# Roy-Shubhajit/FIT-GNN

Measured on AMD Instinct MI355X. Metric: edges aggregated/sec (GCN fwd+bwd) on coarsened subgraphs, higher is better.
Workload: dtype f32

## Files before the change

### fit-gnn_amd/csrc/gcn_ops.hip

```cpp
#include <hip/hip_runtime.h>
#include <stdint.h>

#include <algorithm>

#include "common.h"
#include "fitgnn_hip.h"

namespace {

__global__ void gcn_deg_kernel(const int32_t *__restrict__ rowptr, const float *__restrict__ w, float *__restrict__ dinv,
                               int32_t n_rows) {
    const int i = blockIdx.x * blockDim.x + threadIdx.x;
    if (i >= n_rows) return;
    const int e0 = rowptr[i], e1 = rowptr[i + 1];
    float d = 0.f;
    if (w) {
        for (int e = e0; e < e1; ++e) d += w[e];
    } else {
        d = (float)(e1 - e0);
    }
    dinv[i] = d > 0.f ? 1.0f / sqrtf(d) : 0.f;
}

__global__ void gcn_val_kernel(const int32_t *__restrict__ rowptr, const int32_t *__restrict__ col,
// ... 73 lines not shown
                for (int u = 0; u < U; ++u) nz[u] = __ballot((__float_as_uint(dyl[u]) & 0x7fffffffu) != 0u) != 0ull;
            }
#pragma unroll
            for (int u = 0; u < U; ++u) {
                const int row = min(row0 + 4 * u, r1 - 1);
                const int64_t base = ((sel && !compact_in) ? sel[row] : (int64_t)row) * H + col0;
                if (HEAD && !nz[u]) {
#pragma unroll
                    for (int i = 0; i < VEC; ++i) o[u][i] = 0.f;
                    continue;
                }
                if (VEC == 4) {
                    const float4 ov = *reinterpret_cast<const float4 *>(out + base);
                    o[u][0] = ov.x; o[u][1 % VEC] = ov.y; o[u][2 % VEC] = ov.z; o[u][3 % VEC] = ov.w;
                    if (!HEAD) {
                        const float4 gv = *reinterpret_cast<const float4 *>(dOut + base);
                        g[u][0] = gv.x; g[u][1 % VEC] = gv.y; g[u][2 % VEC] = gv.z; g[u][3 % VEC] = gv.w;
                    }
                } else {
                    o[u][0] = out[base];
                    if (!HEAD) g[u][0] = dOut[base];
                }
            }
#pragma unroll
            for (int u = 0; u < U; ++u) {
                const int row = row0 + 4 * u;
                if (row >= r1) break;
                const int64_t zbase = (int64_t)row * H + col0;
                const int64_t base = (sel ? sel[row] : (int64_t)row) * H + col0;
                if (HEAD && !nz[u]) {
                    if (VEC == 4) {
                        *reinterpret_cast<float4 *>(dZ + zbase) = make_float4(0.f, 0.f, 0.f, 0.f);
                    } else {
                        dZ[zbase] = 0.f;
                    }
                    continue;
                }
                if (HEAD) {
#pragma unroll
                    for (int i = 0; i < VEC; ++i) g[u][i] = 0.f;
                    for (int c = 0; c < C; ++c) {
                        const float d = __int_as_float(__builtin_amdgcn_readlane(__float_as_int(dyl[u]), c));
#pragma unroll
                        for (int i = 0; i < VEC; ++i) g[u][i] = fmaf(d, s_w[c * SLAB + lane * VEC + i], g[u][i]);
                    }
                    if (CW > 0) {
#pragma unroll
                        for (int c = 0; c < (CW > 0 ? CW : 1); ++c) {
                            const float d = __int_as_float(__builtin_amdgcn_readlane(__float_as_int(dyl[u]), c));
#pragma unroll
                            for (int i = 0; i < VEC; ++i) wacc[c][i] = fmaf(d, o[u][i], wacc[c][i]);
                        }
                    }
                }
                uint64_t bits = 0;
                if ((epi & FITGNN_EPI_DROPOUT) && !mask) bits = fitgnn::dropout_bits(seed, (uint64_t)base >> 2);
#pragma unroll
                for (int i = 0; i < VEC; ++i) {
                    float d = g[u][i];
                    if (epi & FITGNN_EPI_DROPOUT) {
                        const uint64_t idx = (uint64_t)base + i;
                        const bool keep = mask ? (mask[idx] != 0) : fitgnn::dropout_keep(bits, (int)(idx & 3), thresh);
                        d = keep ? d * scale : 0.f;
                    }
                    if (epi & FITGNN_EPI_ELU) {
                        const float e = o[u][i] * unscale;
                        d = e > 0.f ? d : d * (e + 1.0f);
// ... 849 lines not shown
```

### fit-gnn_amd/csrc/gemm_f32.hip

```cpp
#include <algorithm>
#include <cmath>

#include "common.h"
#include "fitgnn_hip.h"

namespace {

typedef float f32x16 __attribute__((ext_vector_type(16)));

constexpr int kBK = 32;
constexpr int kPitch = 36;

template <int WM, int WN, int MI, int NJ, bool AKM, bool BKM>
struct Geo {
    static constexpr int TI = 32 * MI * WM, TJ = 32 * NJ * WN, THREADS = 64 * WM * WN;
    static constexpr int A_DW = AKM ? kBK * TI : TI * kPitch;
    static constexpr int B_DW = BKM ? kBK * TJ : TJ * kPitch;
    static constexpr int STAGE_DW = A_DW + B_DW;
    static constexpr int LDS_BYTES = 2 * STAGE_DW * 4;
    static constexpr int NA = TI * 8 / THREADS, NB = TJ * 8 / THREADS;
    static_assert(LDS_BYTES <= 160 * 1024, "tile does not fit the CU's LDS");
    static_assert(TI * 8 % THREADS == 0 && TJ * 8 % THREADS == 0, "stage not divisible over the threads");
};

template <bool KM, int T, int NV, int THREADS>
__device__ __forceinline__ void load_slab(float4 (&r)[NV], const float *__restrict__ P, long ld, long t0, long lim, long k0, long klim) {
    const int tid = threadIdx.x;
#pragma unroll
    for (int p = 0; p < NV; ++p) {
        const int v = tid + p * THREADS;
        if (!KM) {
            const int row = v >> 3, k4 = v & 7;
            long i = t0 + row;
            i = i < lim ? i : lim - 1;
            const long k = k0 + 4 * k4;
            r[p] = k < klim ? *reinterpret_cast<const float4 *>(P + i * ld + k) : make_float4(0.f, 0.f, 0.f, 0.f);
        } else {
            constexpr int Q = T / 4;
            const int kr = v / Q, c4 = v % Q;
            long i = t0 + 4 * c4;
            i = i + 4 <= lim ? i : lim - 4;
            const long k = k0 + kr;
            r[p] = k < klim ? *reinterpret_cast<const float4 *>(P + k * ld + i) : make_float4(0.f, 0.f, 0.f, 0.f);
        }
// ... 9 lines not shown
        if (!KM) {
            const int row = v >> 3, k4 = v & 7;
            *reinterpret_cast<float4 *>(lds + row * kPitch + 4 * k4) = r[p];
        } else {
            constexpr int Q = T / 4;
            const int kr = v / Q, c4 = v % Q;
            *reinterpret_cast<float4 *>(lds + kr * T + 4 * c4) = r[p];
        }
    }
}

template <bool KM, int T>
__device__ __forceinline__ void frag(float (&f)[4], const float *lds, int o, int kk, int lane) {
    if (!KM) {
        const float4 v = *reinterpret_cast<const float4 *>(lds + (o + (lane & 31)) * kPitch + 8 * kk + 4 * (lane >> 5));
        f[0] = v.x; f[1] = v.y; f[2] = v.z; f[3] = v.w;
    } else {
        const float *p = lds + (8 * kk + 4 * (lane >> 5)) * T + o + (lane & 31);
#pragma unroll
        for (int s = 0; s < 4; ++s) f[s] = p[s * T];
    }
}

template <int WM, int WN, int MI, int NJ, bool AKM, bool BKM>
__global__ __launch_bounds__(64 * WM * WN) void gemm_f32_kernel(const float *__restrict__ A, long lda, const float *__restrict__ B, long ldb,
                                                                   long I, int J, long K, float *__restrict__ C, long ldc, int tiles_i,
                                                                   int tiles_j, int nchunks, long chunk_k) {
    using G = Geo<WM, WN, MI, NJ, AKM, BKM>;
    extern __shared__ __attribute__((aligned(16))) float lds_f[];
    const int lane = threadIdx.x & 63, wave = __builtin_amdgcn_readfirstlane(threadIdx.x >> 6);
    const int wm = wave / WN, wn = wave % WN;
    const int xcd = blockIdx.x & 7, slot = blockIdx.x >> 3;
    int ti, tj, chunk = 0;
    if (nchunks > 1) {
        const int ntile = tiles_i * tiles_j;
        const int tile = slot % ntile;
        chunk = xcd + 8 * (slot / ntile);
        ti = tile / tiles_j, tj = tile % tiles_j;
        if (chunk >= nchunks) return;
    } else {
        tj = slot % tiles_j;
        ti = xcd + 8 * (slot / tiles_j);
        if (ti >= tiles_i) return;
    }
    const long i0 = (long)ti * G::TI, j0 = (long)tj * G::TJ;
    const long k_begin = (long)chunk * chunk_k;
    const long k_end = nchunks > 1 ? (k_begin + chunk_k < K ? k_begin + chunk_k : K) : K;
    const int nstage = k_end > k_begin ? (int)((k_end - k_begin + kBK - 1) / kBK) : 0;

    f32x16 acc[MI][NJ];
// ... 34 lines not shown
#pragma unroll
        for (int kk = 0; kk < NKK; ++kk) {
            float fa[MI][4], fb[NJ][4];
            read_frags(fa, fb, sa, sb, kk);
            multiply(fa, fb);
        }
    };
    for (int s = 0; s < nstage; ++s) {
        const bool more = s + 1 < nstage;
        if (more) {
            const long k0 = k_begin + (long)(s + 1) * kBK;
            load_slab<AKM, G::TI, G::NA, G::THREADS>(ra, A, lda, i0, I, k0, k_end);
            load_slab<BKM, G::TJ, G::NB, G::THREADS>(rb, B, ldb, j0, (long)J, k0, k_end);
        }
        products(s);
        if (more) {
            float *na = lds_f + ((s + 1) & 1) * G::STAGE_DW;
            store_slab<AKM, G::TI, G::NA, G::THREADS>(ra, na);
            store_slab<BKM, G::TJ, G::NB, G::THREADS>(rb, na + G::A_DW);
        }
        __syncthreads();
    }

    float *out = nchunks > 1 ? C + (long)chunk * I * J : C;
    const long ldo = nchunks > 1 ? (long)J : ldc;
#pragma unroll
    for (int i = 0; i < MI; ++i) {
#pragma unroll
        for (int j = 0; j < NJ; ++j) {
            const long col = j0 + wn * (32 * NJ) + j * 32 + (lane & 31);
            const long row0 = i0 + wm * (32 * MI) + i * 32 + 4 * (lane >> 5);
#pragma unroll
            for (int r = 0; r < 16; ++r) {
                const long row = row0 + (r & 3) + 8 * (r >> 2);
                if (row < I && col < J) out[row * ldo + col] = acc[i][j][r];
            }
        }
    }
}

__global__ __launch_bounds__(256) void sum_chunks_kernel(const float *__restrict__ partial, int nchunks, long IJ, float *__restrict__ out, int J,
                                                         long ldc) {
    const long q = (long)blockIdx.x * blockDim.x + threadIdx.x;
    if (q >= IJ) return;
    float part[8];
#pragma unroll
    for (int u = 0; u < 8; ++u) part[u] = 0.f;
    int c = 0;
    for (; c + 8 <= nchunks; c += 8) {
#pragma unroll
        for (int u = 0; u < 8; ++u) part[u] += partial[(long)(c + u) * IJ + q];
    }
#pragma unroll
    for (int u = 0; u < 8; ++u)
        if (c + u < nchunks) part[u] += partial[(long)(c + u) * IJ + q];
    float acc = part[0];
#pragma unroll
    for (int u = 1; u < 8; ++u) acc += part[u];
    out[(q / J) * ldc + (q % J)] = acc;
}

enum Shape { S256 = 0, S256x128, S64x512, S128, S64x128, S128x64, S64x64 };
struct ShapeDim { int ti, tj, per_cu; };
constexpr ShapeDim kShape[] = {{256, 256, 1}, {256, 128, 1}, {64, 512, 1}, {128, 128, 2}, {64, 128, 2}, {128, 64, 2}, {64, 64, 4}};

struct Plan {
    int shape;
    int tiles_i, tiles_j, nchunks;
    long chunk_k;
    long main_rows;
    int rem_tiles_i, rem_chunks;
    long rem_chunk_k;
};

Plan make_plan(long I, int J, long K, bool akm, bool bkm) {
    Plan p;
    const bool tn = akm && bkm;
    auto tiles_of = [&](int sh) { return ((I + kShape[sh].ti - 1) / kShape[sh].ti) * ((J + kShape[sh].tj - 1) / kShape[sh].tj); };
    if (tn) {
        if (I <= 64) p.shape = S64x512;
        else if (J <= 128 || K < 65536) p.shape = S128;
        else p.shape = S256;
// ... 26 lines not shown
    for (long c = 8; c <= most && c <= 256; c += 8) {
        const double t = ceil(ntile * (double)c / slots) * t_tile / (double)c + (double)(c + 1) * (double)I * (double)J * 4.0 / 3.0e12 + 4e-6;
        if (t < 0.92 * best) { best = t; p.nchunks = (int)c; }
    }
    if (p.nchunks > 1) {
        const long per = (K + p.nchunks - 1) / p.nchunks;
        p.chunk_k = (per + kBK - 1) / kBK * kBK;
    }
    p.main_rows = 0; p.rem_tiles_i = 0; p.rem_chunks = 1; p.rem_chunk_k = K;
    const long T = (long)p.tiles_i * p.tiles_j;
    const long full = T / 256, rem = T % 256;
    if (!akm && kShape[p.shape].per_cu == 1 && p.nchunks == 1 && full >= 1 && rem > 0 && rem <= 96 && K >= 8 * 2 * kBK) {
        const long main_tiles_i = full * 256 / p.tiles_j;
        if (main_tiles_i >= 1 && main_tiles_i < p.tiles_i) {
            p.main_rows = main_tiles_i * TI;
            p.rem_tiles_i = (int)(p.tiles_i - main_tiles_i);
            p.rem_chunks = 8;
            p.rem_chunk_k = ((K + 7) / 8 + kBK - 1) / kBK * kBK;
        }
    }
    return p;
}

template <int WM, int WN, int MI, int NJ, bool AKM, bool BKM>
int launch(const Plan &p, const float *a, long lda, const float *b, long ldb, long I, int J, long K, float *c, long ldc, hipStream_t s) {
    using G = Geo<WM, WN, MI, NJ, AKM, BKM>;
    static std::atomic<uint64_t> lds_done{0};
    if (const int rc = fitgnn_lds_limit_once((const void *)gemm_f32_kernel<WM, WN, MI, NJ, AKM, BKM>, G::LDS_BYTES, lds_done)) return rc;
    unsigned grid;
    if (p.nchunks > 1) grid = (unsigned)(p.tiles_i * p.tiles_j * ((p.nchunks + 7) / 8 * 8));
    else grid = (unsigned)((p.tiles_i + 7) / 8 * 8 * p.tiles_j);
    hipLaunchKernelGGL((gemm_f32_kernel<WM, WN, MI, NJ, AKM, BKM>), dim3(grid), dim3(G::THREADS), G::LDS_BYTES, s, a, lda, b, ldb, I, J, K,
                       c, ldc, p.tiles_i, p.tiles_j, p.nchunks, p.chunk_k);
    return (int)hipGetLastError();
}

template <bool AKM, bool BKM>
int launch_shape(const Plan &p, const float *a, long lda, const float *b, long ldb, long I, int J, long K, float *c, long ldc, hipStream_t s) {
    if constexpr (AKM && BKM) {
        if (p.shape == S64x512) return launch<1, 4, 2, 4, AKM, BKM>(p, a, lda, b, ldb, I, J, K, c, ldc, s);
    }
    switch (p.shape) {
        case S256x128: return launch<4, 1, 2, 4, AKM, BKM>(p, a, lda, b, ldb, I, J, K, c, ldc, s);
        case S128: return launch<2, 2, 2, 2, AKM, BKM>(p, a, lda, b, ldb, I, J, K, c, ldc, s);
        case S64x128: return launch<2, 2, 1, 2, AKM, BKM>(p, a, lda, b, ldb, I, J, K, c, ldc, s);
        case S128x64: return launch<4, 1, 1, 2, AKM, BKM>(p, a, lda, b, ldb, I, J, K, c, ldc, s);
        case S64x64: return launch<2, 2, 1, 1, AKM, BKM>(p, a, lda, b, ldb, I, J, K, c, ldc, s);
        default: return launch<4, 2, 2, 4, AKM, BKM>(p, a, lda, b, ldb, I, J, K, c, ldc, s);
    }
}

}

extern "C" size_t fitgnn_gemm_exact_workspace_bytes(int64_t I, int32_t J, int64_t K, int32_t a_kmajor, int32_t b_kmajor) {
    if (I <= 0 || J <= 0 || K <= 0) return 0;
    const Plan p = make_plan((long)I, J, (long)K, a_kmajor != 0, b_kmajor != 0);
    if (p.main_rows > 0) return (size_t)p.rem_chunks * (size_t)(I - p.main_rows) * (size_t)J * sizeof(float);
    return p.nchunks > 1 ? (size_t)p.nchunks * (size_t)I * (size_t)J * sizeof(float) : 0;
}

extern "C" int fitgnn_gemm_exact_plan(int64_t I, int32_t J, int64_t K, int32_t a_kmajor, int32_t b_kmajor, int32_t *shape, int32_t *nchunks,
                                      int64_t *main_rows) {
    if (I <= 0 || J <= 0 || K <= 0 || !shape || !nchunks || !main_rows) return FITGNN_E_BADARG;
    const Plan p = make_plan((long)I, J, (long)K, a_kmajor != 0, b_kmajor != 0);
    *shape = p.shape;
    *nchunks = p.nchunks;
    *main_rows = p.main_rows;
    return 0;
}

extern "C" int fitgnn_gemm_exact_f32(const float *a, int64_t lda, int32_t a_kmajor, const float *b, int64_t ldb, int32_t b_kmajor,
                                     int64_t I, int32_t J, int64_t K, float *c, int64_t ldc, void *workspace, void *stream) {
// ... 27 lines not shown
        hipLaunchKernelGGL(sum_chunks_kernel, dim3((unsigned)((IJ + 255) / 256)), dim3(256), 0, s, (const float *)workspace, pr.nchunks, IJ,
                           c + p.main_rows * (long)ldc, J, (long)ldc);
        return (int)hipGetLastError();
    }
    float *dst = c;
    long ldd = (long)ldc;
    if (p.nchunks > 1) {
        if (!workspace || ((uintptr_t)workspace % 16) != 0) return FITGNN_E_BADARG;
        dst = (float *)workspace;
    }
    int rc;
    if (a_kmajor) rc = launch_shape<true, true>(p, a, (long)lda, b, (long)ldb, (long)I, J, (long)K, dst, ldd, s);
    else if (b_kmajor) rc = launch_shape<false, true>(p, a, (long)lda, b, (long)ldb, (long)I, J, (long)K, dst, ldd, s);
    else rc = launch_shape<false, false>(p, a, (long)lda, b, (long)ldb, (long)I, J, (long)K, dst, ldd, s);
    if (rc) return rc;
    if (p.nchunks > 1) {
        const long IJ = (long)I * J;
        hipLaunchKernelGGL(sum_chunks_kernel, dim3((unsigned)((IJ + 255) / 256)), dim3(256), 0, s, (const float *)workspace, p.nchunks, IJ, c, J,
                           (long)ldc);
        return (int)hipGetLastError();
    }
    return 0;
}
```

### fit-gnn_amd/fitgnn_amd/_lib.py

```python
import ctypes
import os

_HERE = os.path.dirname(os.path.abspath(__file__))
LIB_PATH = os.path.join(os.path.dirname(_HERE), "lib", "libfitgnn_hip.so")

c_i32, c_i64, c_u32, c_u64, c_f32, c_size = (ctypes.c_int32, ctypes.c_int64, ctypes.c_uint32, ctypes.c_uint64,
                                              ctypes.c_float, ctypes.c_size_t)
ptr = ctypes.c_void_p

EPI_BIAS, EPI_ELU, EPI_DROPOUT, EPI_SEED_DEVICE = 1, 2, 4, 8
SPMM_GATHER = 0x100
MAX_K = 16
MATCH_HEAVY_EDGE, MATCH_ALGEBRAIC_JC = 0, 1
MATCH_SMALL_MAX_NODES, MATCH_SMALL_MAX_NNZ, MATCH_SMALL_MAX_K, MATCH_SMALL_LDS_BUDGET = 128, 1024, 12, 65536
MATCH_DONE, MATCH_TOO_BIG, MATCH_BAD_INPUT = 1, 2, 3
QUALITY_MAX_K = 64

SIGNATURES = {
    "fitgnn_abi_version": (ctypes.c_int, []),
    "fitgnn_error_string": (ctypes.c_char_p, [ctypes.c_int]),
    "fitgnn_stream_copy_f32": (ctypes.c_int, [ptr, ptr, c_i64, ptr]),
    "fitgnn_spmm_default_window_rows": (ctypes.c_int, []),
    "fitgnn_spmm_max_window_rows": (ctypes.c_int, [c_i32]),
    "fitgnn_gcn_norm_csr_f32": (ctypes.c_int, [ptr, ptr, ptr, ptr, ptr, c_i32, ptr]),
# ... 40 lines not shown
    "fitgnn_epilogue_bwd_head_rows_f32": (ctypes.c_int, [ptr, ptr, c_i32, ptr, ptr, c_i32, c_i32, ptr, c_i32, c_u32, c_f32, c_u64, ptr,
                                                        ptr, ptr, ptr, c_size, ptr]),
    "fitgnn_epilogue_bwd_rows_f32": (ctypes.c_int, [ptr, ptr, ptr, c_i32, c_i32, ptr, c_i32, c_u32, c_f32, c_u64, ptr, ptr, ptr, c_size, ptr]),
    "fitgnn_spmm_epilogue_bwd_supported": (ctypes.c_int, [c_i32, c_i32, c_i32]),
    "fitgnn_spmm_epilogue_bwd_workspace_bytes": (c_size, [c_i32, c_i32, c_i32]),
    "fitgnn_spmm_epilogue_bwd_f32": (ctypes.c_int, [ptr, ptr, ptr, ptr, c_i32, c_i32, ptr, ptr, ptr, c_i32, ptr, ptr, c_i32, c_i32,
                                                   c_u32, c_f32, c_u64, ptr, ptr, ptr, ptr, c_size, ptr]),
    "fitgnn_gat_scores_f32": (ctypes.c_int, [ptr, c_i64, c_i32, c_i32, ptr, ptr, ptr, ptr, ptr]),
    "fitgnn_gat_edge_softmax_f32": (ctypes.c_int, [ptr, ptr, ptr, ptr, c_f32, c_i32, ptr, ptr]),
    "fitgnn_sddmm_csr_f32": (ctypes.c_int, [ptr, ptr, ptr, c_i64, ptr, c_i64, c_i32, c_i32, ptr, ptr]),
    "fitgnn_sddmm_csr_rows_f32": (ctypes.c_int, [ptr, ptr, ptr, c_i64, ptr, c_i64, ptr, c_i32, c_i32, ptr, ptr]),
    "fitgnn_gat_softmax_bwd_rows_f32": (ctypes.c_int, [ptr, ptr, ptr, ptr, ptr, ptr, c_f32, ptr, c_i32, ptr, ptr, ptr]),
    "fitgnn_gat_softmax_bwd_f32": (ctypes.c_int, [ptr, ptr, ptr, ptr, ptr, ptr, c_f32, c_i32, ptr, ptr, ptr]),
    "fitgnn_l1_loss_f32": (ctypes.c_int, [ptr, ptr, c_i32, c_f32, ptr, ptr, ptr]),
    "fitgnn_softmax_nll_workspace_bytes": (c_size, [c_i32]),
    "fitgnn_softmax_nll_f32": (ctypes.c_int, [ptr, c_i64, c_i32, c_i32, ptr, ptr, c_i32, c_f32, ptr, ptr, ptr, c_size, ptr]),
    "fitgnn_adam_step_f32": (ctypes.c_int, [ptr, ptr, ptr, ptr, c_i64, c_f32, c_f32, c_f32, c_f32, c_f32, ptr, ptr]),
    "fitgnn_sum_leading_f32": (ctypes.c_int, [ptr, c_i32, c_i64, ptr, ptr]),
    "fitgnn_gemm_atb_workspace_bytes": (c_size, [c_i64, c_i32, c_i32]),
    "fitgnn_gemm_atb_f32": (ctypes.c_int, [ptr, c_i64, ptr, c_i64, c_i64, c_i32, c_i32, ptr, ptr, ptr]),
    "fitgnn_gemm_nt_f32": (ctypes.c_int, [ptr, c_i64, ptr, c_i64, c_i64, c_i32, c_i32, ptr, c_i64, ptr]),
    "fitgnn_gemm_exact_workspace_bytes": (c_size, [c_i64, c_i32, c_i64, c_i32, c_i32]),
    "fitgnn_gemm_exact_f32": (ctypes.c_int, [ptr, c_i64, c_i32, ptr, c_i64, c_i32, c_i64, c_i32, c_i64, ptr, c_i64, ptr, ptr]),
    "fitgnn_gemm_exact_plan": (ctypes.c_int, [c_i64, c_i32, c_i64, c_i32, c_i32, ptr, ptr, ptr]),
    "fitgnn_gemm_nt_presplit_bytes": (c_size, [c_i32, c_i32]),
    "fitgnn_gemm_nt_presplit_f32": (ctypes.c_int, [ptr, c_i64, c_i64, c_i32, c_i32, c_i32, ptr, ptr]),
    "fitgnn_gemm_nt_pre_f32": (ctypes.c_int, [ptr, c_i64, ptr, c_i64, c_i32, c_i32, ptr, c_i64, ptr]),
    "fitgnn_gemm_nt_epilogue_bwd_workspace_bytes": (c_size, [c_i64, c_i32]),
    "fitgnn_gemm_nt_epilogue_bwd_f32": (ctypes.c_int, [ptr, c_i64, ptr, c_i64, c_i64, c_i32, c_i32, ptr, ptr, ctypes.c_uint32, c_f32,
                                                       ctypes.c_uint64, ptr, ptr, ptr, c_size, ptr]),
    "fitgnn_colsum_partials_f32": (ctypes.c_int, [ptr, c_i32, c_i32, ptr, ptr]),
    "fitgnn_head_rows_lds_bytes": (c_size, [c_i32, c_i32]),
    "fitgnn_head_rows_f32": (ctypes.c_int, [ptr, c_i64, ptr, c_i32, ptr, ptr, c_i32, c_i32, ptr, c_i64, c_i32, ptr]),
    "fitgnn_epilogue_fwd_rows_f32": (ctypes.c_int, [ptr, c_i64, ptr, c_i32, c_i32, ptr, c_u32, c_f32, c_u64, ptr, ptr]),
    "fitgnn_dense_narrow_k_lds_bytes": (c_size, [c_i32, c_i32]),
    "fitgnn_dense_narrow_k_f32": (ctypes.c_int, [ptr, c_i64, ptr, c_i64, c_i32, c_i32, c_i32, ptr, c_u32, c_f32, c_u64, ptr, ptr, c_i64, ptr]),
    "fitgnn_narrow_atb_workspace_bytes": (c_size, [c_i32, c_i32, c_i32]),
    "fitgnn_narrow_atb_f32": (ctypes.c_int, [ptr, c_i64, ptr, c_u32, c_f32, c_u64, ptr, ptr, c_i64, c_i32, c_i32, c_i32, ptr, ptr, ptr, c_size,
                                             ptr]),
    "fitgnn_adam_step_acc_f32": (ctypes.c_int, [ptr, ptr, ptr, ptr, ptr, c_i64, c_f32, c_f32, c_f32, c_f32, c_f32, ptr, ptr, c_i32, c_u64, ptr]),
    "fitgnn_pool_head_supported": (ctypes.c_int, [c_i32, c_i32]),
    "fitgnn_pool_head_f32": (ctypes.c_int, [ptr, ptr, c_i32, ptr, c_i64, c_i32, ptr, ptr, ptr, c_i32, ptr, ptr, ptr]),
    "fitgnn_pool_head_bwd_f32": (ctypes.c_int, [ptr, ptr, c_i32, ptr, ptr, ptr, c_i64, c_i32, c_i32, ptr, ptr, ptr, ptr]),
    "fitgnn_colsum_narrow_workspace_bytes": (c_size, [c_i32, c_i32]),
    "fitgnn_colsum_narrow_f32": (ctypes.c_int, [ptr, c_i64, c_i32, c_i32, ptr, ptr, c_size, ptr]),
    "fitgnn_spmm_narrow_f32": (ctypes.c_int, [ptr, ptr, ptr, ptr, ptr, c_i32, c_i32, c_f32, ptr, c_f32, ptr, c_f32, ptr]),
# ... 109 lines not shown
```

### fit-gnn_amd/fitgnn_amd/ops.py

```python
import ctypes

import os

import torch

from . import _lib
from ._lib import EPI_BIAS, EPI_DROPOUT, EPI_ELU


class OpConfig:
    __slots__ = ("gemm_precision", "atb_kernel", "nt_kernel", "nt_presplit", "fuse_dx_epilogue", "fold_backward",
                 "dedup_gather", "pad_table_min_k", "split_large_blocks", "compact_head_backward", "last_layer_on_loss_rows",
                 "compact_rows_kernel", "stream_kernel", "two_hop_backward", "narrow_input_first", "fused_pool_head", "pooled_rows_last_layer", "rows_kernel_min_rows", "appnp_in_lds", "appnp_blocks", "appnp_sliced", "grad_sink", "profile", "profile_gemm",
                 "profile_fused", "seed_bank")

    def __init__(self, gemm_precision="exact", atb_kernel=True, nt_kernel=True, nt_presplit=True, fuse_dx_epilogue=True,
                 fold_backward=False, dedup_gather=True, pad_table_min_k=0, split_large_blocks=True, compact_head_backward=True,
                 last_layer_on_loss_rows=True, compact_rows_kernel=True, stream_kernel=False, two_hop_backward=True, narrow_input_first=True, fused_pool_head=True, pooled_rows_last_layer=True, rows_kernel_min_rows=32768, appnp_in_lds=True, appnp_blocks=True, appnp_sliced=True, grad_sink=None,
                 profile=None, profile_gemm=None, profile_fused=None, seed_bank=None):
        if gemm_precision not in ("exact", "high", "highest"):
            raise ValueError(f"gemm_precision {gemm_precision!r}: 'exact', 'high' or 'highest'")
        self.gemm_precision, self.atb_kernel, self.nt_kernel, self.nt_presplit = gemm_precision, atb_kernel, nt_kernel, nt_presplit
        self.fuse_dx_epilogue, self.fold_backward, self.dedup_gather = fuse_dx_epilogue, fold_backward, dedup_gather
        self.pad_table_min_k, self.split_large_blocks = pad_table_min_k, split_large_blocks
        self.compact_head_backward, self.last_layer_on_loss_rows = compact_head_backward, last_layer_on_loss_rows
        self.compact_rows_kernel, self.stream_kernel, self.two_hop_backward = compact_rows_kernel, stream_kernel, two_hop_backward
        self.narrow_input_first, self.fused_pool_head, self.grad_sink = narrow_input_first, fused_pool_head, grad_sink
        self.pooled_rows_last_layer, self.rows_kernel_min_rows = pooled_rows_last_layer, int(rows_kernel_min_rows)
        self.appnp_in_lds, self.appnp_blocks, self.appnp_sliced = appnp_in_lds, appnp_blocks, appnp_sliced
        self.profile, self.profile_gemm, self.profile_fused, self.seed_bank = profile, profile_gemm, profile_fused, seed_bank

    def replace(self, **kw):
        cur = {k: getattr(self, k) for k in self.__slots__}
        cur.update(kw)
        return OpConfig(**cur)


DEFAULT = OpConfig()


def _addresses(*params):
    return tuple(None if t is None else t.data_ptr() for t in params)


class _GradSink:
    __slots__ = ("_sink", "_slices")

    def __init__(self, grad_sink):
        self._sink, self._slices = grad_sink, []

    def slice(self, ptr):
        if self._sink is None or ptr is None:
            return None
# ... 27 lines not shown
    L = _lib.lib()
    if form == "nt":
        (I, K), J, akm, bkm = a.shape, b.shape[0], 0, 0
        assert b.shape[1] == K
    elif form == "nn":
        (I, K), J, akm, bkm = a.shape, b.shape[1], 0, 1
        assert b.shape[0] == K
    elif form == "tn":
        (K, I), J, akm, bkm = a.shape, b.shape[1], 1, 1
        assert b.shape[0] == K
    else:
        raise ValueError(form)
    if out is None:
        out = torch.empty((I, J), dtype=torch.float32, device=a.device)
    else:
        assert out.shape == (I, J) and out.dtype == torch.float32 and out.stride(1) == 1 and out.is_cuda
    wb = int(L.fitgnn_gemm_exact_workspace_bytes(I, J, K, akm, bkm))
    ws = torch.empty(wb // 4, dtype=torch.float32, device=a.device) if wb else None
    ev = _gemm_events(cfg, "gemm_f32_kernel[%s]" % form, 2.0 * I * J * K)
    rc = L.fitgnn_gemm_exact_f32(_lib.dptr(a), a.stride(0), akm, _lib.dptr(b), b.stride(0), bkm, I, J, K, _lib.dptr(out), out.stride(0),
                                 _lib.dptr(ws), _lib.stream_ptr(a.device))
    _gemm_done(cfg, ev)
    _lib.check(rc, "fitgnn_gemm_exact_f32")
    return out


def padded_weight(W, Kp):
    Wp = torch.zeros((W.shape[0], Kp), dtype=torch.float32, device=W.device)
    Wp[:, : W.shape[1]] = W
    return Wp


def _full_grid(R, N):
    return ((R + 255) // 256) * ((N + 255) // 256) >= 128


def _nt_ok(a, b, cfg):
    if not (cfg.nt_kernel and cfg.gemm_precision == "high" and a.is_cuda and a.dtype == torch.float32 and b.dtype == torch.float32
            and a.dim() == 2 and b.dim() == 2 and a.stride(1) == 1 and a.shape[1] % 32 == 0 and a.shape[0] >= 1024
            and b.shape[0] >= 64 and a.stride(0) % 4 == 0 and a.data_ptr() % 16 == 0):
        return False
    if cfg.nt_presplit and _full_grid(a.shape[0], b.shape[0]):
        return True
    return b.stride(1) == 1 and b.stride(0) % 4 == 0 and b.data_ptr() % 16 == 0


# ... 1241 lines not shown
    @staticmethod
    def backward(ctx, dy):
        X, W, Wl, out, mask = ctx.saved_tensors
        dy = _f32c(dy)
        cfg, ep = ctx.cfg, ctx.ep
        dH, db, dWl = layer_backward(ctx.g, out, ep.bwd, ep.p, ep.seed, mask, ctx.has_bias, dy=dy, Wl=Wl, want_dWl=ctx.needs_input_grad[3],
                                     cfg=cfg, loss_rows=ctx.loss_rows)
        dy_l = dy if ctx.loss_rows is None else dy.index_select(0, ctx.loss_rows)
        dbl = colsum_narrow(dy_l) if ctx.has_bl and ctx.needs_input_grad[4] else None
        dW = mm_at_b(dH, X, cfg) if ctx.needs_input_grad[1] else None
        dX = _dx_through_link(cfg, ctx.link_in, dH, W, X) if ctx.needs_input_grad[0] else None
        return dX, dW, (db if ctx.has_bias else None), dWl, dbl, None, None, None, None, None, None, None, None


def _arange_rows(g, n, device):
    cache = getattr(g, "_arange_rows", None)
    if cache is None or cache.numel() != n or cache.device != device:
        cache = torch.arange(n, dtype=torch.int64, device=device)
        g._arange_rows = cache
    return cache


def _dense_rows(AHc, W, b, rows, ep, cfg):
    outc = mm_xwt(AHc, W, cfg)
    if not outc.is_contiguous():
        outc = outc.contiguous()
    return epilogue_fwd_rows_(outc, rows, b, ep.fwd, p=ep.p, seed=ep.seed, mask=ep.mask)


def _head_rows_fwd(outc, Wl, bl, rows, n_total, compact_out, g, cfg):
    if _exact(cfg, outc, Wl) and Wl.shape[0] >= 16:
        y = gemm_exact(outc, Wl, "nt", cfg)
        if bl is not None:
            y = y + bl
        if not compact_out:
            y = torch.zeros((n_total, y.shape[1]), dtype=torch.float32, device=y.device).index_copy_(0, rows, y)
        return y
    if compact_out:
        return head_rows(outc, _arange_rows(g, rows.numel(), rows.device), Wl, bl, n_total=rows.numel())
    return head_rows(outc, rows, Wl, bl, n_total=n_total)


def _head_rows_bwd(dy, rows, compact_out, outc, Wl, ep, mask, has_bias, want_dWl, want_dbl, cfg, sink, pb=None, pWl=None, pbl=None):
    H, C = outc.shape[1], Wl.shape[0]
    dy_c = _f32c(dy) if compact_out else _f32c(dy).index_select(0, rows)
    inside = want_dWl and bool(_lib.lib().fitgnn_epilogue_bwd_head_supported(H, C, 1))
# ... 671 lines not shown
```

### include/fitgnn_hip.h

```cpp
#ifndef FITGNN_HIP_H
#define FITGNN_HIP_H

#include <stddef.h>
#include <stdint.h>

#ifdef __cplusplus
extern "C" {
#endif

#define FITGNN_ABI_VERSION 1
#define FITGNN_MAX_K 16

#define FITGNN_E_BADARG (-1)
#define FITGNN_E_WORKSPACE (-2)
#define FITGNN_E_ALIGN (-3)

int fitgnn_abi_version(void);
const char *fitgnn_error_string(int code);

int fitgnn_stream_copy_f32(const float *src, float *dst, int64_t n, void *stream);


typedef struct fitgnn_tile {
    int32_t row_begin, row_end;
// ... 101 lines not shown
                              void *stream);

int fitgnn_pool_head_supported(int32_t F, int32_t C);
int fitgnn_pool_head_f32(const int32_t *seg_off, const int32_t *members, int32_t n_seg, const float *X, int64_t ldx, int32_t F,
                         const float *inv_cnt, const float *W, const float *b, int32_t C, float *pooled, float *y, void *stream);
int fitgnn_pool_head_bwd_f32(const float *dy, const float *W, int32_t C, const float *pooled, const int32_t *seg_of_row,
                             const float *inv_cnt, int64_t n_rows, int32_t n_seg, int32_t F, float *dx, float *dW, float *db,
                             void *stream);

int fitgnn_sum_leading_f32(const float *part, int32_t B, int64_t W, float *out, void *stream);

size_t fitgnn_gemm_atb_workspace_bytes(int64_t R, int32_t M, int32_t N);
int fitgnn_gemm_atb_f32(const float *a, int64_t lda, const float *b, int64_t ldb, int64_t R, int32_t M, int32_t N,
                        float *out, void *workspace, void *stream);

int fitgnn_gemm_nt_f32(const float *a, int64_t lda, const float *b, int64_t ldb, int64_t R, int32_t N, int32_t K,
                       float *c, int64_t ldc, void *stream);

size_t fitgnn_gemm_exact_workspace_bytes(int64_t I, int32_t J, int64_t K, int32_t a_kmajor, int32_t b_kmajor);
int fitgnn_gemm_exact_f32(const float *a, int64_t lda, int32_t a_kmajor, const float *b, int64_t ldb, int32_t b_kmajor,
                          int64_t I, int32_t J, int64_t K, float *c, int64_t ldc, void *workspace, void *stream);
int fitgnn_gemm_exact_plan(int64_t I, int32_t J, int64_t K, int32_t a_kmajor, int32_t b_kmajor, int32_t *shape, int32_t *nchunks,
                           int64_t *main_rows);

size_t fitgnn_gemm_nt_presplit_bytes(int32_t N, int32_t K);
int fitgnn_gemm_nt_presplit_f32(const float *b, int64_t stride_n, int64_t stride_k, int32_t N, int32_t K, int32_t K_valid,
                                void *image, void *stream);
int fitgnn_gemm_nt_pre_f32(const float *a, int64_t lda, const void *b_image, int64_t R, int32_t N, int32_t K, float *c,
                           int64_t ldc, void *stream);

size_t fitgnn_gemm_nt_epilogue_bwd_workspace_bytes(int64_t R, int32_t N);
int fitgnn_gemm_nt_epilogue_bwd_f32(const float *a, int64_t lda, const float *b, int64_t ldb, int64_t R, int32_t N, int32_t K,
                                    const float *out, float *dZ, uint32_t epilogue, float p_drop, uint64_t seed,
                                    const uint8_t *mask, float *db, void *work, size_t work_bytes, void *stream);

size_t fitgnn_head_rows_lds_bytes(int32_t H, int32_t C);
int fitgnn_head_rows_f32(const float *out, int64_t ldo, const int64_t *rows, int32_t n_rows, const float *Wl, const float *bl,
                         int32_t C, int32_t H, float *y, int64_t ldy, int32_t out_compact, void *stream);

size_t fitgnn_colsum_narrow_workspace_bytes(int32_t n_rows, int32_t C);
int fitgnn_colsum_narrow_f32(const float *x, int64_t ldx, int32_t n_rows, int32_t C, float *out, void *work, size_t work_bytes,
                             void *stream);

int fitgnn_colsum_partials_f32(const float *partial, int32_t n_chunks, int32_t H, float *out, void *stream);

int fitgnn_l1_loss_f32(const float *out, const float *tgt, int32_t n, float scale, float *loss, float *grad, void *stream);
// ... 236 lines not shown
```

Before: 3.666 billion.

## Fuse bias/ELU/dropout epilogue into exact GEMM store and batch head-row FMAs

Adds an epilogue variant of the exact f32 GEMM. The accumulator tile is staged through per-wave LDS regions and bias, ELU and dropout are applied as it is stored, with a separate pass for split-K and remainder rows. _dense_rows uses this path by default, so the separate elementwise pass over the dense output and its extra memory traffic go away. Separately, the head backward kernel processes all U rows together when every row is nonzero, loading each weight slab value from LDS once per class instead of once per row. The costs are more template instantiations and LDS reuse for draining tiles, and the dropout index must match the unfused path to give identical results.

```diff
diff --git a/fit-gnn_amd/csrc/gcn_ops.hip b/fit-gnn_amd/csrc/gcn_ops.hip
--- a/fit-gnn_amd/csrc/gcn_ops.hip
+++ b/fit-gnn_amd/csrc/gcn_ops.hip
@@ -119,6 +119,29 @@
                     if (!HEAD) g[u][0] = dOut[base];
                 }
             }
+            bool joint = false;
+            if (HEAD) {
+                joint = true;
+#pragma unroll
+                for (int u = 0; u < U; ++u) joint = joint && nz[u];
+                if (joint) {
+#pragma unroll
+                    for (int u = 0; u < U; ++u)
+#pragma unroll
+                        for (int i = 0; i < VEC; ++i) g[u][i] = 0.f;
+                    for (int c = 0; c < C; ++c) {
+                        float w[VEC];
+#pragma unroll
+                        for (int i = 0; i < VEC; ++i) w[i] = s_w[c * SLAB + lane * VEC + i];
+#pragma unroll
+                        for (int u = 0; u < U; ++u) {
+                            const float d = __int_as_float(__builtin_amdgcn_readlane(__float_as_int(dyl[u]), c));
+#pragma unroll
+                            for (int i = 0; i < VEC; ++i) g[u][i] = fmaf(d, w[i], g[u][i]);
+                        }
+                    }
+                }
+            }
 #pragma unroll
             for (int u = 0; u < U; ++u) {
                 const int row = row0 + 4 * u;
@@ -134,12 +157,14 @@
                     continue;
                 }
                 if (HEAD) {
-#pragma unroll
-                    for (int i = 0; i < VEC; ++i) g[u][i] = 0.f;
-                    for (int c = 0; c < C; ++c) {
-                        const float d = __int_as_float(__builtin_amdgcn_readlane(__float_as_int(dyl[u]), c));
-#pragma unroll
-                        for (int i = 0; i < VEC; ++i) g[u][i] = fmaf(d, s_w[c * SLAB + lane * VEC + i], g[u][i]);
+                    if (!joint) {
+#pragma unroll
+                        for (int i = 0; i < VEC; ++i) g[u][i] = 0.f;
+                        for (int c = 0; c < C; ++c) {
+                            const float d = __int_as_float(__builtin_amdgcn_readlane(__float_as_int(dyl[u]), c));
+#pragma unroll
+                            for (int i = 0; i < VEC; ++i) g[u][i] = fmaf(d, s_w[c * SLAB + lane * VEC + i], g[u][i]);
+                        }
                     }
                     if (CW > 0) {
 #pragma unroll
diff --git a/fit-gnn_amd/csrc/gemm_f32.hip b/fit-gnn_amd/csrc/gemm_f32.hip
--- a/fit-gnn_amd/csrc/gemm_f32.hip
+++ b/fit-gnn_amd/csrc/gemm_f32.hip
@@ -19,7 +19,10 @@
     static constexpr int STAGE_DW = A_DW + B_DW;
     static constexpr int LDS_BYTES = 2 * STAGE_DW * 4;
     static constexpr int NA = TI * 8 / THREADS, NB = TJ * 8 / THREADS;
+    static constexpr int DRAIN_PITCH = 32 * NJ + 8;
+    static constexpr int DRAIN_DW = 32 * DRAIN_PITCH;
     static_assert(LDS_BYTES <= 160 * 1024, "tile does not fit the CU's LDS");
+    static_assert(AKM || BKM || WM * WN * DRAIN_DW * 4 <= LDS_BYTES, "drain regions do not fit the stage buffers");
     static_assert(TI * 8 % THREADS == 0 && TJ * 8 % THREADS == 0, "stage not divisible over the threads");
 };
 
@@ -75,10 +78,38 @@
     }
 }
 
-template <int WM, int WN, int MI, int NJ, bool AKM, bool BKM>
+struct EpiArgs {
+    const int64_t *rows;
+    const float *bias;
+    const uint8_t *mask;
+    uint64_t seed;
+    uint32_t flags;
+    float p_drop;
+};
+
+__device__ __forceinline__ float4 epi_apply4(float4 v, int64_t orow, int col0, int H, const EpiArgs &ep, uint64_t seed, float keep_scale,
+                                             uint32_t thresh) {
+    float x[4] = {v.x, v.y, v.z, v.w};
+    const uint64_t idx0 = (uint64_t)orow * (uint64_t)H + (uint64_t)col0;
+    uint64_t bits = 0;
+    if ((ep.flags & FITGNN_EPI_DROPOUT) && !ep.mask) bits = fitgnn::dropout_bits(seed, idx0 >> 2);
+#pragma unroll
+    for (int e = 0; e < 4; ++e) {
+        float y = x[e] + ((ep.flags & FITGNN_EPI_BIAS) ? ep.bias[col0 + e] : 0.f);
+        if (ep.flags & FITGNN_EPI_ELU) y = y > 0.f ? y : __expf(y) - 1.0f;
+        if (ep.flags & FITGNN_EPI_DROPOUT) {
+            const bool keep = ep.mask ? (ep.mask[idx0 + e] != 0) : fitgnn::dropout_keep(bits, (int)((idx0 + e) & 3), thresh);
+            y = keep ? y * keep_scale : 0.f;
+        }
+        x[e] = y;
+    }
+    return make_float4(x[0], x[1], x[2], x[3]);
+}
+
+template <int WM, int WN, int MI, int NJ, bool AKM, bool BKM, bool EPI = false>
 __global__ __launch_bounds__(64 * WM * WN) void gemm_f32_kernel(const float *__restrict__ A, long lda, const float *__restrict__ B, long ldb,
                                                                    long I, int J, long K, float *__restrict__ C, long ldc, int tiles_i,
-                                                                   int tiles_j, int nchunks, long chunk_k) {
+                                                                   int tiles_j, int nchunks, long chunk_k, EpiArgs ep) {
     using G = Geo<WM, WN, MI, NJ, AKM, BKM>;
     extern __shared__ __attribute__((aligned(16))) float lds_f[];
     const int lane = threadIdx.x & 63, wave = __builtin_amdgcn_readfirstlane(threadIdx.x >> 6);
@@ -159,6 +190,40 @@
         __syncthreads();
     }
 
+    if constexpr (EPI) {
+        const uint64_t seed = fitgnn::resolve_seed(ep.seed, ep.flags);
+        const float keep_scale = (ep.flags & FITGNN_EPI_DROPOUT) ? 1.0f / (1.0f - ep.p_drop) : 1.0f;
+        const uint32_t thresh = fitgnn::dropout_threshold(ep.p_drop);
+        float *dr = lds_f + wave * G::DRAIN_DW;
+        constexpr int P = G::DRAIN_PITCH, Q = 8 * NJ;
+#pragma unroll
+        for (int i = 0; i < MI; ++i) {
+#pragma unroll
+            for (int j = 0; j < NJ; ++j)
+#pragma unroll
+                for (int r = 0; r < 16; ++r)
+                    dr[((r & 3) + 8 * (r >> 2) + 4 * (lane >> 5)) * P + j * 32 + (lane & 31)] = acc[i][j][r];
+            __builtin_amdgcn_fence(__ATOMIC_RELEASE, "wavefront");
+            __builtin_amdgcn_wave_barrier();
+            const long rbase = i0 + wm * (32 * MI) + i * 32;
+            const int cbase = (int)j0 + wn * (32 * NJ);
+#pragma unroll 4
+            for (int it = 0; it < 32 * Q / 64; ++it) {
+                const int v = it * 64 + lane;
+                const int rl = v / Q, c4 = v % Q;
+                const long row = rbase + rl;
+                const int col = cbase + 4 * c4;
+                if (row < I && col < J) {
+                    const float4 a4 = *reinterpret_cast<const float4 *>(dr + rl * P + 4 * c4);
+                    const int64_t orow = ep.rows ? ep.rows[row] : (int64_t)row;
+                    *reinterpret_cast<float4 *>(C + row * ldc + col) = epi_apply4(a4, orow, col, J, ep, seed, keep_scale, thresh);
+                }
+            }
+            __builtin_amdgcn_fence(__ATOMIC_RELEASE, "wavefront");
+            __builtin_amdgcn_wave_barrier();
+        }
+        return;
+    }
     float *out = nchunks > 1 ? C + (long)chunk * I * J : C;
     const long ldo = nchunks > 1 ? (long)J : ldc;
 #pragma unroll
@@ -195,6 +260,21 @@
 #pragma unroll
     for (int u = 1; u < 8; ++u) acc += part[u];
     out[(q / J) * ldc + (q % J)] = acc;
+}
+
+__global__ __launch_bounds__(256) void epi_rows_kernel(float *__restrict__ z, long ldz, long row0, long n, int H, EpiArgs ep) {
+    const uint64_t seed = fitgnn::resolve_seed(ep.seed, ep.flags);
+    const float keep_scale = (ep.flags & FITGNN_EPI_DROPOUT) ? 1.0f / (1.0f - ep.p_drop) : 1.0f;
+    const uint32_t thresh = fitgnn::dropout_threshold(ep.p_drop);
+    const int H4 = H >> 2;
+    const long total = n * H4;
+    for (long t = (long)blockIdx.x * 256 + threadIdx.x; t < total; t += (long)gridDim.x * 256) {
+        const long i = t / H4;
+        const int col0 = (int)(t - i * H4) * 4;
+        const int64_t orow = ep.rows ? ep.rows[row0 + i] : (int64_t)(row0 + i);
+        float4 *p = reinterpret_cast<float4 *>(z + i * ldz + col0);
+        *p = epi_apply4(*p, orow, col0, H, ep, seed, keep_scale, thresh);
+    }
 }
 
 enum Shape { S256 = 0, S256x128, S64x512, S128, S64x128, S128x64, S64x64 };
@@ -267,16 +347,17 @@
     return p;
 }
 
-template <int WM, int WN, int MI, int NJ, bool AKM, bool BKM>
-int launch(const Plan &p, const float *a, long lda, const float *b, long ldb, long I, int J, long K, float *c, long ldc, hipStream_t s) {
+template <int WM, int WN, int MI, int NJ, bool AKM, bool BKM, bool EPI = false>
+int launch(const Plan &p, const float *a, long lda, const float *b, long ldb, long I, int J, long K, float *c, long ldc, hipStream_t s,
+           const EpiArgs &ep = EpiArgs{}) {
     using G = Geo<WM, WN, MI, NJ, AKM, BKM>;
     static std::atomic<uint64_t> lds_done{0};
-    if (const int rc = fitgnn_lds_limit_once((const void *)gemm_f32_kernel<WM, WN, MI, NJ, AKM, BKM>, G::LDS_BYTES, lds_done)) return rc;
+    if (const int rc = fitgnn_lds_limit_once((const void *)gemm_f32_kernel<WM, WN, MI, NJ, AKM, BKM, EPI>, G::LDS_BYTES, lds_done)) return rc;
     unsigned grid;
     if (p.nchunks > 1) grid = (unsigned)(p.tiles_i * p.tiles_j * ((p.nchunks + 7) / 8 * 8));
     else grid = (unsigned)((p.tiles_i + 7) / 8 * 8 * p.tiles_j);
-    hipLaunchKernelGGL((gemm_f32_kernel<WM, WN, MI, NJ, AKM, BKM>), dim3(grid), dim3(G::THREADS), G::LDS_BYTES, s, a, lda, b, ldb, I, J, K,
-                       c, ldc, p.tiles_i, p.tiles_j, p.nchunks, p.chunk_k);
+    hipLaunchKernelGGL((gemm_f32_kernel<WM, WN, MI, NJ, AKM, BKM, EPI>), dim3(grid), dim3(G::THREADS), G::LDS_BYTES, s, a, lda, b, ldb, I, J,
+                       K, c, ldc, p.tiles_i, p.tiles_j, p.nchunks, p.chunk_k, ep);
     return (int)hipGetLastError();
 }
 
@@ -293,6 +374,25 @@
         case S64x64: return launch<2, 2, 1, 1, AKM, BKM>(p, a, lda, b, ldb, I, J, K, c, ldc, s);
         default: return launch<4, 2, 2, 4, AKM, BKM>(p, a, lda, b, ldb, I, J, K, c, ldc, s);
     }
+}
+
+int launch_shape_epi(const Plan &p, const float *a, long lda, const float *b, long ldb, long I, int J, long K, float *c, long ldc, hipStream_t s,
+                     const EpiArgs &ep) {
+    switch (p.shape) {
+        case S256x128: return launch<4, 1, 2, 4, false, false, true>(p, a, lda, b, ldb, I, J, K, c, ldc, s, ep);
+        case S128: return launch<2, 2, 2, 2, false, false, true>(p, a, lda, b, ldb, I, J, K, c, ldc, s, ep);
+        case S64x128: return launch<2, 2, 1, 2, false, false, true>(p, a, lda, b, ldb, I, J, K, c, ldc, s, ep);
+        case S128x64: return launch<4, 1, 1, 2, false, false, true>(p, a, lda, b, ldb, I, J, K, c, ldc, s, ep);
+        case S64x64: return launch<2, 2, 1, 1, false, false, true>(p, a, lda, b, ldb, I, J, K, c, ldc, s, ep);
+        default: return launch<4, 2, 2, 4, false, false, true>(p, a, lda, b, ldb, I, J, K, c, ldc, s, ep);
+    }
+}
+
+int launch_epi_rows(float *z, long ldz, long row0, long n, int H, const EpiArgs &ep, hipStream_t s) {
+    const long total = n * (H / 4);
+    const int blocks = (int)std::min<long>((total + 255) / 256, 256 * 16);
+    hipLaunchKernelGGL(epi_rows_kernel, dim3(blocks), dim3(256), 0, s, z, ldz, row0, n, H, ep);
+    return (int)hipGetLastError();
 }
 
 }
@@ -366,3 +466,38 @@
     }
     return 0;
 }
+
+extern "C" int fitgnn_gemm_exact_epi_f32(const float *a, int64_t lda, const float *b, int64_t ldb, int64_t I, int32_t J, int64_t K, float *c,
+                                         int64_t ldc, const int64_t *rows, const float *bias, uint32_t epilogue, float p_drop, uint64_t seed,
+                                         const uint8_t *mask, void *workspace, void *stream) {
+    if (I <= 0 || J < 4 || (J % 4) != 0 || K < 4 || (K % 4) != 0 || ldc < J || (ldc % 4) != 0) return FITGNN_E_BADARG;
+    if (!a || !b || !c || lda < K || ldb < K || (lda % 4) != 0 || (ldb % 4) != 0) return FITGNN_E_BADARG;
+    if ((epilogue & FITGNN_EPI_BIAS) && !bias) return FITGNN_E_BADARG;
+    if ((epilogue & FITGNN_EPI_DROPOUT) && !(p_drop >= 0.f && p_drop < 1.f)) return FITGNN_E_BADARG;
+    if ((((uintptr_t)a | (uintptr_t)b | (uintptr_t)c) % 16) != 0) return FITGNN_E_ALIGN;
+    const Plan p = make_plan((long)I, J, (long)K, false, false);
+    hipStream_t s = (hipStream_t)stream;
+    const EpiArgs ep{rows, bias, mask, seed, epilogue, p_drop};
+    if (p.nchunks > 1) {
+        const int rc = fitgnn_gemm_exact_f32(a, lda, 0, b, ldb, 0, I, J, K, c, ldc, workspace, stream);
+        return rc ? rc : launch_epi_rows(c, (long)ldc, 0, (long)I, J, ep, s);
+    }
+    if (p.main_rows > 0) {
+        if (!workspace || ((uintptr_t)workspace % 16) != 0) return FITGNN_E_BADARG;
+        Plan pm = p, pr = p;
+        pm.tiles_i = (int)(p.main_rows / kShape[p.shape].ti);
+        pr.tiles_i = p.rem_tiles_i; pr.nchunks = p.rem_chunks; pr.chunk_k = p.rem_chunk_k;
+        const long rem_rows = (long)I - p.main_rows;
+        int rc = launch_shape_epi(pm, a, (long)lda, b, (long)ldb, p.main_rows, J, (long)K, c, (long)ldc, s, ep);
+        if (!rc)
+            rc = launch_shape<false, false>(pr, a + p.main_rows * (long)lda, (long)lda, b, (long)ldb, rem_rows, J, (long)K, (float *)workspace,
+                                            (long)J, s);
+        if (rc) return rc;
+        const long IJ = rem_rows * J;
+        float *c_rem = c + p.main_rows * (long)ldc;
+        hipLaunchKernelGGL(sum_chunks_kernel, dim3((unsigned)((IJ + 255) / 256)), dim3(256), 0, s, (const float *)workspace, pr.nchunks, IJ, c_rem,
+                           J, (long)ldc);
+        return launch_epi_rows(c_rem, (long)ldc, p.main_rows, rem_rows, J, ep, s);
+    }
+    return launch_shape_epi(p, a, (long)lda, b, (long)ldb, (long)I, J, (long)K, c, (long)ldc, s, ep);
+}
diff --git a/fit-gnn_amd/fitgnn_amd/_lib.py b/fit-gnn_amd/fitgnn_amd/_lib.py
--- a/fit-gnn_amd/fitgnn_amd/_lib.py
+++ b/fit-gnn_amd/fitgnn_amd/_lib.py
@@ -86,6 +86,8 @@
     "fitgnn_gemm_nt_f32": (ctypes.c_int, [ptr, c_i64, ptr, c_i64, c_i64, c_i32, c_i32, ptr, c_i64, ptr]),
     "fitgnn_gemm_exact_workspace_bytes": (c_size, [c_i64, c_i32, c_i64, c_i32, c_i32]),
     "fitgnn_gemm_exact_f32": (ctypes.c_int, [ptr, c_i64, c_i32, ptr, c_i64, c_i32, c_i64, c_i32, c_i64, ptr, c_i64, ptr, ptr]),
+    "fitgnn_gemm_exact_epi_f32": (ctypes.c_int, [ptr, c_i64, ptr, c_i64, c_i64, c_i32, c_i64, ptr, c_i64, ptr, ptr, c_u32, c_f32, c_u64, ptr, ptr,
+                                                 ptr]),
     "fitgnn_gemm_exact_plan": (ctypes.c_int, [c_i64, c_i32, c_i64, c_i32, c_i32, ptr, ptr, ptr]),
     "fitgnn_gemm_nt_presplit_bytes": (c_size, [c_i32, c_i32]),
     "fitgnn_gemm_nt_presplit_f32": (ctypes.c_int, [ptr, c_i64, c_i64, c_i32, c_i32, c_i32, ptr, ptr]),
diff --git a/fit-gnn_amd/fitgnn_amd/ops.py b/fit-gnn_amd/fitgnn_amd/ops.py
--- a/fit-gnn_amd/fitgnn_amd/ops.py
+++ b/fit-gnn_amd/fitgnn_amd/ops.py
@@ -11,12 +11,12 @@
 class OpConfig:
     __slots__ = ("gemm_precision", "atb_kernel", "nt_kernel", "nt_presplit", "fuse_dx_epilogue", "fold_backward",
                  "dedup_gather", "pad_table_min_k", "split_large_blocks", "compact_head_backward", "last_layer_on_loss_rows",
-                 "compact_rows_kernel", "stream_kernel", "two_hop_backward", "narrow_input_first", "fused_pool_head", "pooled_rows_last_layer", "rows_kernel_min_rows", "appnp_in_lds", "appnp_blocks", "appnp_sliced", "grad_sink", "profile", "profile_gemm",
+                 "compact_rows_kernel", "stream_kernel", "two_hop_backward", "narrow_input_first", "fused_pool_head", "gemm_store_epilogue", "pooled_rows_last_layer", "rows_kernel_min_rows", "appnp_in_lds", "appnp_blocks", "appnp_sliced", "grad_sink", "profile", "profile_gemm",
                  "profile_fused", "seed_bank")
 
     def __init__(self, gemm_precision="exact", atb_kernel=True, nt_kernel=True, nt_presplit=True, fuse_dx_epilogue=True,
                  fold_backward=False, dedup_gather=True, pad_table_min_k=0, split_large_blocks=True, compact_head_backward=True,
-                 last_layer_on_loss_rows=True, compact_rows_kernel=True, stream_kernel=False, two_hop_backward=True, narrow_input_first=True, fused_pool_head=True, pooled_rows_last_layer=True, rows_kernel_min_rows=32768, appnp_in_lds=True, appnp_blocks=True, appnp_sliced=True, grad_sink=None,
+                 last_layer_on_loss_rows=True, compact_rows_kernel=True, stream_kernel=False, two_hop_backward=True, narrow_input_first=True, fused_pool_head=True, gemm_store_epilogue=True, pooled_rows_last_layer=True, rows_kernel_min_rows=32768, appnp_in_lds=True, appnp_blocks=True, appnp_sliced=True, grad_sink=None,
                  profile=None, profile_gemm=None, profile_fused=None, seed_bank=None):
         if gemm_precision not in ("exact", "high", "highest"):
             raise ValueError(f"gemm_precision {gemm_precision!r}: 'exact', 'high' or 'highest'")
@@ -29,6 +29,7 @@
         self.pooled_rows_last_layer, self.rows_kernel_min_rows = pooled_rows_last_layer, int(rows_kernel_min_rows)
         self.appnp_in_lds, self.appnp_blocks, self.appnp_sliced = appnp_in_lds, appnp_blocks, appnp_sliced
         self.profile, self.profile_gemm, self.profile_fused, self.seed_bank = profile, profile_gemm, profile_fused, seed_bank
+        self.gemm_store_epilogue = gemm_store_epilogue
 
     def replace(self, **kw):
         cur = {k: getattr(self, k) for k in self.__slots__}
@@ -102,6 +103,30 @@
                                  _lib.dptr(ws), _lib.stream_ptr(a.device))
     _gemm_done(cfg, ev)
     _lib.check(rc, "fitgnn_gemm_exact_f32")
+    return out
+
+
+def gemm_exact_epi(a, b, rows, bias, epilogue, p=0.0, seed=0, mask=None, cfg=DEFAULT, out=None):
+    L = _lib.lib()
+    (I, K), J = a.shape, b.shape[0]
+    assert b.shape[1] == K and J % 4 == 0
+    _lib.require_cuda(a, b, rows, bias, mask)
+    if out is None:
+        out = torch.empty((I, J), dtype=torch.float32, device=a.device)
+    else:
+        assert out.shape == (I, J) and out.dtype == torch.float32 and out.stride(1) == 1 and out.stride(0) % 4 == 0 and out.is_cuda
+    seed, epilogue = _seed_arg(seed, epilogue)
+    if rows is not None:
+        rows = (rows if rows.dtype == torch.int64 else rows.long()).contiguous()
+        assert rows.numel() == I
+    wb = int(L.fitgnn_gemm_exact_workspace_bytes(I, J, K, 0, 0))
+    ws = torch.empty(wb // 4, dtype=torch.float32, device=a.device) if wb else None
+    ev = _gemm_events(cfg, "gemm_f32_kernel[nt]", 2.0 * I * J * K)
+    rc = L.fitgnn_gemm_exact_epi_f32(_lib.dptr(a), a.stride(0), _lib.dptr(b), b.stride(0), I, J, K, _lib.dptr(out), out.stride(0),
+                                     _lib.dptr(rows), _lib.dptr(None if bias is None else _f32c(bias)), epilogue, float(p), seed,
+                                     _lib.dptr(mask), _lib.dptr(ws), _lib.stream_ptr(a.device))
+    _gemm_done(cfg, ev)
+    _lib.check(rc, "fitgnn_gemm_exact_epi_f32")
     return out
 
 
@@ -1389,6 +1414,8 @@
 
 
 def _dense_rows(AHc, W, b, rows, ep, cfg):
+    if cfg.gemm_store_epilogue and _exact(cfg, AHc, W) and W.shape[0] % 4 == 0:
+        return gemm_exact_epi(AHc, W, rows, b, ep.fwd, p=ep.p, seed=ep.seed, mask=ep.mask, cfg=cfg)
     outc = mm_xwt(AHc, W, cfg)
     if not outc.is_contiguous():
         outc = outc.contiguous()
diff --git a/include/fitgnn_hip.h b/include/fitgnn_hip.h
--- a/include/fitgnn_hip.h
+++ b/include/fitgnn_hip.h
@@ -147,6 +147,10 @@
                           int64_t I, int32_t J, int64_t K, float *c, int64_t ldc, void *workspace, void *stream);
 int fitgnn_gemm_exact_plan(int64_t I, int32_t J, int64_t K, int32_t a_kmajor, int32_t b_kmajor, int32_t *shape, int32_t *nchunks,
                            int64_t *main_rows);
+
+int fitgnn_gemm_exact_epi_f32(const float *a, int64_t lda, const float *b, int64_t ldb, int64_t I, int32_t J, int64_t K, float *c,
+                              int64_t ldc, const int64_t *rows, const float *bias, uint32_t epilogue, float p_drop, uint64_t seed,
+                              const uint8_t *mask, void *workspace, void *stream);
 
 size_t fitgnn_gemm_nt_presplit_bytes(int32_t N, int32_t K);
 int fitgnn_gemm_nt_presplit_f32(const float *b, int64_t stride_n, int64_t stride_k, int32_t N, int32_t K, int32_t K_valid,
```

Result: no change. 3.684 billion, median of 6 (+0.5%).
